# DistributedML/Biscotti

Measured on AMD Instinct MI355X. Metric: Multi-Krum GB/s (device-resident, n fp64 updates x d) + selected-set parity, higher is better.
Workload: dtype f64; 1 GPU; D_512x1M_f153; n=512, d=1048576, f=153, m=359, parallelism=1 GPU, d_local=1048576

## Files before the change

### biscotti_amd/csrc/bk_kernels.hip

```cpp
#include <hip/hip_runtime.h>
#include <stdint.h>
#include <stdlib.h>
#include <string.h>
#include <type_traits>

#include "bk_device.h"
#include "bk_internal.h"
#include "bk_synth.h"

namespace bk {

typedef float f2v __attribute__((ext_vector_type(2)));
typedef double d4v __attribute__((ext_vector_type(4)));


__device__ __forceinline__ int xcd_remap(int b, int nwg) {
    const int q = nwg >> 3, r = nwg & 7, x = b & 7;
    return (x < r ? x * (q + 1) : r * (q + 1) + (x - r) * q) + (b >> 3);
}

__device__ __forceinline__ void tri_decode(int u, int T, int &bi, int &bj) {
    int i = 0, off = 0;
    while (u >= off + (T - i)) { off += T - i; ++i; }
    bi = i;
// ... 224 lines not shown
    case 11: asm volatile("s_waitcnt vmcnt(11)" ::: "memory"); break;
    default: asm volatile("s_waitcnt vmcnt(12)" ::: "memory"); break;
    }
}

template <int N>
__device__ __forceinline__ void g3_waitc() {
    asm volatile("s_waitcnt vmcnt(%0)" ::"n"(N) : "memory");
}

__device__ __forceinline__ void g3_barrier() {
    __builtin_amdgcn_s_barrier();
    asm volatile("" ::: "memory");
    __builtin_amdgcn_sched_barrier(0);
}

__device__ __forceinline__ constexpr int dix(int i, int j) { return i * 4 - i * (i - 1) / 2 + (j - i); }

template <int KIND, typename V>
struct G3Acc;
template <typename V>
struct G3Acc<T_OFF, V> {
    V a[4][4];
};
template <typename V>
struct G3Acc<T_PAIR, V> {
    V a[10], b[10];
};
template <typename V>
struct G3Acc<T_DIAG1, V> {
    V a[10];
};

template <typename T, bool SKIP = false>
__device__ __forceinline__ void diag_mma(typename G3T<T>::acc (&acc)[10], const d2v (&a)[4]) {
    typedef typename G3T<T>::op O;
#pragma unroll
    for (int s = 0; s < 2; ++s)
#pragma unroll
        for (int i = 0; i < 4; ++i)
#pragma unroll
            for (int j = i; j < 4; ++j) {
                if (SKIP && i == 0 && j == 3) continue;
                acc[dix(i, j)] = G3T<T>::mma((O)a[i][s], (O)a[j][s], acc[dix(i, j)]);
            }
}
template <typename T>
__device__ __forceinline__ void off_mma_tail(typename G3T<T>::acc (&acc)[4][4], const d2v (&a)[4],
                                             const d2v (&b)[4]) {
    typedef typename G3T<T>::op O;
#pragma unroll
    for (int s = 0; s < 2; ++s)
#pragma unroll
        for (int i = 0; i < 4; ++i)
#pragma unroll
            for (int j = 0; j < 4; ++j) acc[i][j] = G3T<T>::mma((O)a[i][s], (O)b[j][s], acc[i][j]);
}
template <typename T, bool SKIP = false>
__device__ __forceinline__ void diag_mma_g(typename G3T<T>::acc (&acc)[10],
                                           const typename G3T<T>::gran (&a)[4]) {
#pragma unroll
    for (int s = 0; s < G3T<T>::SUB; ++s) {
        typename G3T<T>::op v[4];
#pragma unroll
        for (int i = 0; i < 4; ++i) v[i] = G3T<T>::at(a[i], s);
#pragma unroll
        for (int i = 0; i < 4; ++i)
#pragma unroll
            for (int j = i; j < 4; ++j) {
                if (SKIP && i == 0 && j == 3) continue;
                acc[dix(i, j)] = G3T<T>::mma(v[i], v[j], acc[dix(i, j)]);
            }
    }
}

template <typename T>
__device__ __forceinline__ void g3_load_rows(d2v (&a)[4], const T *__restrict__ X, int64_t ld,
                                             int n, int b, int64_t c, int64_t d, int rr) {
#pragma unroll
    for (int q = 0; q < 4; ++q) {
        const T *pr = X + (int64_t)min(b * 64 + q * 16 + rr, n - 1) * ld;
        a[q].x = c < d ? (double)pr[c] : 0.0;
        a[q].y = c + 1 < d ? (double)pr[c + 1] : 0.0;
    }
}

template <typename T = double>
__device__ __forceinline__ void store_tile(double *out, const typename G3T<T>::acc (&acc)[4][4],
                                           int rr, int g, bool wt = false) {
#pragma unroll
    for (int i = 0; i < 4; ++i)
#pragma unroll
        for (int j = 0; j < 4; ++j)
#pragma unroll
            for (int r = 0; r < 4; ++r)
                st_part(&out[(i * 16 + g3_crow<T>(g, r)) * 64 + j * 16 + rr], (double)acc[i][j][r], wt);
}

template <typename T, bool SKIP = false>
__device__ __forceinline__ void store_diag(double *out, const typename G3T<T>::acc (&acc)[10],
                                           int rr, int g, bool wt = false) {
#pragma unroll
    for (int i = 0; i < 4; ++i)
#pragma unroll
        for (int j = 0; j < 4; ++j) {
            if (SKIP && i == 0 && j == 3) continue;
#pragma unroll
            for (int r = 0; r < 4; ++r)
                st_part(&out[(i * 16 + g3_crow<T>(g, r)) * 64 + j * 16 + rr],
                        j >= i ? (double)acc[dix(i, j)][r] : 0.0, wt);
        }
}

template <typename T, int S, int XT = 0>
__device__ __forceinline__ void off_mma(typename G3T<T>::acc (&acc)[4][4],
                                        const typename G3T<T>::gran (&a)[4],
                                        const typename G3T<T>::gran (&b)[4],
                                        typename G3T<T>::acc &x) {
    typename G3T<T>::op va[4], vb[4];
#pragma unroll
    for (int i = 0; i < 4; ++i) {
        va[i] = G3T<T>::at(a[i], S);
        vb[i] = G3T<T>::at(b[i], S);
    }
#pragma unroll
    for (int i = 0; i < 4; ++i)
#pragma unroll
        for (int j = 0; j < 4; ++j)
            acc[i][j] = G3T<T>::mma(va[i], vb[j], acc[i][j]);
    if constexpr (XT == 1) x = G3T<T>::mma(va[0], va[3], x);
    if constexpr (XT == 2) x = G3T<T>::mma(vb[0], vb[3], x);
}
template <typename T, int XT = 0>
__device__ __forceinline__ void off_mma_gran(typename G3T<T>::acc (&acc)[4][4],
                                             const typename G3T<T>::gran (&a)[4],
                                             const typename G3T<T>::gran (&b)[4],
                                             typename G3T<T>::acc &x) {
    off_mma<T, 0, XT>(acc, a, b, x);
    off_mma<T, 1, XT>(acc, a, b, x);
    if constexpr (G3T<T>::SUB == 4) {
        off_mma<T, 2, XT>(acc, a, b, x);
        off_mma<T, 3, XT>(acc, a, b, x);
    }
}
#ifdef BK_K1_PROBE
#define G3_PROBE(v) const long long v = (long long)__builtin_readcyclecounter()
#else
#define G3_PROBE(v) const long long v = 0
#endif
template <typename T, int KIND, int MODE, bool STAG, int NB, int XT = 0>
__device__ __forceinline__ void g3_wave(const T *__restrict__ X, int64_t ld, int n, int nfull,
                                        int64_t d, const GroupDesc &G, const int *wd, char *lds,
                                        int wave, int lane, double *out, long long (&probe)[2],
                                        double *xout = nullptr, bool wt = false) {
    constexpr int XO = KIND == T_OFF ? XT : 0;
    constexpr bool XP = KIND == T_PAIR && XT != 0;
    typedef typename G3T<T>::gran gran;
    constexpr int EPG = 16 / (int)sizeof(T);
    constexpr int BKE = 8 * EPG;
    const int rr = lane & 15, g = lane >> 4;
    int blk[G3_MAXB];
#pragma unroll
    for (int b = 0; b < G3_MAXB; ++b) blk[b] = G.blk[b];
    const int c = NB > 0 ? NB : G.nb;
    const int sA = G.task[wave][1], sB = G.task[wave][2];
    const int kst = wd[1], kstr = wd[2], kend = wd[3];
    const int nk = kst < kend ? (kend - 1 - kst) / kstr + 1 : 0;

#ifndef BK_GLDS_E6
#define BK_GLDS_E6 2
#endif
#ifndef BK_GLDS_E4
#define BK_GLDS_E4 2
#endif
    constexpr int ESPL = G3T<T>::F32C ? 0 : NB == 6 ? BK_GLDS_E6 : NB == 4 ? BK_GLDS_E4 : 0;
    constexpr int CLO = NB + ESPL, CHI = NB - ESPL;
    constexpr int GMAX = G3_MAXB + 2;
    static_assert(CLO <= GMAX && CHI >= 0, "glds split exceeds the per-wave pointer table");
    const bool hi = wave >= 4;
    const T *gsrc[GMAX];
    int gdst[GMAX];
    {
        const int rq = lane >> 3, j = lane & 7;
#pragma unroll
        for (int m = 0; m < GMAX; ++m) {
            int i = wave + 8 * m;
            if constexpr (ESPL != 0) {
                i = hi ? 4 * CLO + (wave - 4) + 4 * m : wave + 4 * m;
                if (i >= 8 * NB) i = 0;
            }
            const int b = i >> 3, ii = i & 7;
            const int rl = ii * 8 + rq;
#ifdef BK_K1_SAMEROWS
            const int grow = min(rl, n - 1);
#else
            const int grow = min(blk[b] * 64 + rl, n - 1);
#endif
            gsrc[m] = X + (int64_t)grow * ld + EPG * (j ^ (rl & 7));
            gdst[m] = b * G3_BLK + ii * 1024;
        }
    }
    auto issue = [&](int64_t kb, int stage) {
#ifdef BK_K1_L2WINDOW
        const int64_t col = (kb % BK_K1_L2WINDOW) * BKE;
#else
        const int64_t col = kb * BKE;
#endif
        char *base = lds + stage * G3_STAGE;
#ifndef BK_K1_GLDS_LIMIT
#define BK_K1_GLDS_LIMIT G3_MAXB
#endif
        if constexpr (ESPL != 0) {
            if (hi) {
#pragma unroll
                for (int m = 0; m < CHI; ++m)
                    __builtin_amdgcn_global_load_lds((const void *)(gsrc[m] + col),
                                                     (void *)(base + gdst[m]), 16, 0, 0);
            } else {
#pragma unroll
                for (int m = 0; m < CLO; ++m)
                    __builtin_amdgcn_global_load_lds((const void *)(gsrc[m] + col),
                                                     (void *)(base + gdst[m]), 16, 0, 0);
            }
            return;
        }
#pragma unroll
        for (int m = 0; m < (NB > 0 ? NB : G3_MAXB); ++m)
            if ((NB > 0 || m < c) && m < BK_K1_GLDS_LIMIT)
                __builtin_amdgcn_global_load_lds((const void *)(gsrc[m] + col),
                                                 (void *)(base + gdst[m]), 16, 0, 0);
    };

    typedef typename G3T<T>::acc AV;
    G3Acc<KIND == T_NONE ? T_DIAG1 : KIND, AV> acc;
    if constexpr (KIND == T_OFF) {
#pragma unroll
        for (int i = 0; i < 4; ++i)
#pragma unroll
            for (int j = 0; j < 4; ++j) acc.a[i][j] = AV{0, 0, 0, 0};
    } else if constexpr (KIND == T_PAIR) {
#pragma unroll
        for (int i = 0; i < 10; ++i) acc.a[i] = acc.b[i] = AV{0, 0, 0, 0};
    } else if constexpr (KIND == T_DIAG1) {
#pragma unroll
        for (int i = 0; i < 10; ++i) acc.a[i] = AV{0, 0, 0, 0};
    }
    AV xacc = AV{0, 0, 0, 0};
    gran ha[4], hb[4];
#pragma unroll
    for (int q = 0; q < 4; ++q) ha[q] = hb[q] = gran{};

#pragma unroll
    for (int s = 0; s < G3_STAGES - 1; ++s)
        if (s < nk && MODE != 2) issue(kst + (int64_t)s * kstr, s);
    int buf = 0;
    for (int t = 0; t < nk; ++t) {
        const int ahead = min(nk - t - 1, G3_STAGES - 2);
        G3_PROBE(p0);
        if constexpr (NB > 0 && MODE != 2 && ESPL != 0) {
            if (ahead > 0) {
                if (hi)
                    g3_waitc<CHI>();
                else
                    g3_waitc<CLO>();
            } else {
                g3_waitc<0>();
            }
        } else if constexpr (NB > 0 && MODE != 2) {
            if (ahead > 0)
                g3_waitc<(NB < BK_K1_GLDS_LIMIT ? NB : BK_K1_GLDS_LIMIT)>();
            else
                g3_waitc<0>();
        } else {
            g3_wait(MODE == 2 ? 0 : ahead * c);
        }
        G3_PROBE(p1);
        g3_barrier();
        G3_PROBE(p2);
        probe[0] += p1 - p0;
        probe[1] += p2 - p1;
        const char *ls = lds + buf * G3_STAGE;
        const int nbuf = buf == 0 ? G3_STAGES - 1 : buf - 1;
        const bool more = t + G3_STAGES - 1 < nk && MODE != 2;
        const int64_t nkb = kst + (int64_t)(t + G3_STAGES - 1) * kstr;
        buf = buf == G3_STAGES - 1 ? 0 : buf + 1;
        if constexpr (MODE == 1) {
            if (more) issue(nkb, nbuf);
            continue;
        }
        if constexpr (KIND == T_OFF) {
            gran a0[4], b0[4], a1[4], b1[4];
#pragma unroll
            for (int q = 0; q < 4; ++q) a0[q] = g3_frag<T>(ls + sA * G3_BLK, q, 0, rr, g);
#pragma unroll
            for (int q = 0; q < 4; ++q) b0[q] = g3_frag<T>(ls + sB * G3_BLK, q, 0, rr, g);
            if constexpr (STAG) {
                if (t > 0) off_mma_gran<T, XO>(acc.a, ha, hb, xacc);
            }
#pragma unroll
            for (int q = 0; q < 4; ++q) a1[q] = g3_frag<T>(ls + sA * G3_BLK, q, 1, rr, g);
#pragma unroll
            for (int q = 0; q < 4; ++q) b1[q] = g3_frag<T>(ls + sB * G3_BLK, q, 1, rr, g);
            if (more) issue(nkb, nbuf);
            off_mma_gran<T, XO>(acc.a, a0, b0, xacc);
            if constexpr (STAG) {
#pragma unroll
                for (int q = 0; q < 4; ++q) {
                    ha[q] = a1[q];
                    hb[q] = b1[q];
                }
            } else {
                off_mma_gran<T, XO>(acc.a, a1, b1, xacc);
            }
        } else if constexpr (KIND == T_PAIR) {
#pragma unroll
            for (int h = 0; h < 2; ++h) {
                gran a[4], b[4];
#pragma unroll
                for (int q = 0; q < 4; ++q) a[q] = g3_frag<T>(ls + sA * G3_BLK, q, h, rr, g);
#pragma unroll
                for (int q = 0; q < 4; ++q) b[q] = g3_frag<T>(ls + sB * G3_BLK, q, h, rr, g);
                if (h == 0 && more) issue(nkb, nbuf);
                diag_mma_g<T, XP>(acc.a, a);
                diag_mma_g<T, XP>(acc.b, b);
            }
        } else if constexpr (KIND == T_DIAG1) {
#pragma unroll
            for (int h = 0; h < 2; ++h) {
                gran a[4];
#pragma unroll
                for (int q = 0; q < 4; ++q) a[q] = g3_frag<T>(ls + sA * G3_BLK, q, h, rr, g);
                if (h == 0 && more) issue(nkb, nbuf);
                diag_mma_g<T>(acc.a, a);
            }
        } else {
            if (more) issue(nkb, nbuf);
        }
    }
    if constexpr (KIND == T_OFF && STAG && MODE != 1)
        if (nk > 0) off_mma_gran<T, XO>(acc.a, ha, hb, xacc);
    if constexpr (KIND != T_NONE) {
        const int64_t c0 = (int64_t)nfull * BKE;
        if (wd[4] && c0 < d) {
#pragma unroll
            for (int h = 0; h < BKE / 8; ++h) {
                const int64_t cc = c0 + 8 * h + 2 * g;
                d2v a[4], b[4];
                g3_load_rows<T>(a, X, ld, n, blk[sA], cc, d, rr);
                g3_load_rows<T>(b, X, ld, n, blk[sB], cc, d, rr);
                if constexpr (KIND == T_OFF) {
                    typedef typename G3T<T>::op O;
                    off_mma_tail<T>(acc.a, a, b);
#pragma unroll
                    for (int s2 = 0; s2 < 2; ++s2) {
                        if constexpr (XO == 1) xacc = G3T<T>::mma((O)a[0][s2], (O)a[3][s2], xacc);
                        if constexpr (XO == 2) xacc = G3T<T>::mma((O)b[0][s2], (O)b[3][s2], xacc);
                    }
                } else if constexpr (KIND == T_PAIR) {
                    diag_mma<T, XP>(acc.a, a);
                    diag_mma<T, XP>(acc.b, b);
                } else {
                    diag_mma<T>(acc.a, a);
                }
            }
        }
        if constexpr (KIND == T_OFF) {
            store_tile<T>(out, acc.a, rr, g, wt);
            if constexpr (XO != 0) {
#pragma unroll
                for (int r = 0; r < 4; ++r)
                    st_part(&xout[g3_crow<T>(g, r) * 64 + 48 + rr], (double)xacc[r], wt);
            }
        } else if constexpr (KIND == T_PAIR) {
            store_diag<T, XP>(out, acc.a, rr, g, wt);
            store_diag<T, XP>(out + 4096, acc.b, rr, g, wt);
        } else {
            store_diag<T>(out, acc.a, rr, g, wt);
        }
    }
}

#ifndef G3_STAGGER
#define G3_STAGGER 1
#endif
template <typename T, int MODE, int NB>
__device__ __forceinline__ void g3_dispatch(const T *__restrict__ X, int64_t ld, int n,
                                            int nfull, int64_t d, const GroupDesc &G,
                                            const int *wd, char *lds, int wave, int lane,
                                            double *out, long long (&probe)[2], bool wt) {
    const int xt = (NB == 4 || NB == 0) ? G.xt[wave] : 0;
    double *xout = out - (int64_t)wave * 2 * 4096 + (int64_t)G.xslot[wave] * 4096;
    switch (G.task[wave][0]) {
    case T_OFF:
#ifndef BK_F32_STAGGER
#define BK_F32_STAGGER 0
#endif
        if (wave >= 4 && G3_STAGGER && (!G3T<T>::F32C || BK_F32_STAGGER)) {
            if (xt == 1)
                g3_wave<T, T_OFF, MODE, true, NB, (NB == 4 || NB == 0) ? 1 : 0>(X, ld, n, nfull, d, G, wd, lds, wave, lane, out, probe, xout, wt);
            else if (xt == 2)
                g3_wave<T, T_OFF, MODE, true, NB, (NB == 4 || NB == 0) ? 2 : 0>(X, ld, n, nfull, d, G, wd, lds, wave, lane, out, probe, xout, wt);
            else
                g3_wave<T, T_OFF, MODE, true, NB>(X, ld, n, nfull, d, G, wd, lds, wave, lane, out, probe, nullptr, wt);
        } else {
            if (xt == 1)
                g3_wave<T, T_OFF, MODE, false, NB, (NB == 4 || NB == 0) ? 1 : 0>(X, ld, n, nfull, d, G, wd, lds, wave, lane, out, probe, xout, wt);
            else if (xt == 2)
                g3_wave<T, T_OFF, MODE, false, NB, (NB == 4 || NB == 0) ? 2 : 0>(X, ld, n, nfull, d, G, wd, lds, wave, lane, out, probe, xout, wt);
            else
                g3_wave<T, T_OFF, MODE, false, NB>(X, ld, n, nfull, d, G, wd, lds, wave, lane, out, probe, nullptr, wt);
        }
        break;
    case T_PAIR:
        if (xt)
            g3_wave<T, T_PAIR, MODE, false, NB, (NB == 4 || NB == 0) ? 1 : 0>(X, ld, n, nfull, d, G, wd, lds, wave, lane, out, probe, nullptr, wt);
        else
            g3_wave<T, T_PAIR, MODE, false, NB>(X, ld, n, nfull, d, G, wd, lds, wave, lane, out, probe, nullptr, wt);
        break;
    case T_DIAG1:
        g3_wave<T, T_DIAG1, MODE, false, NB>(X, ld, n, nfull, d, G, wd, lds, wave, lane, out, probe, nullptr, wt);
        break;
    default:
        g3_wave<T, T_NONE, MODE, false, NB>(X, ld, n, nfull, d, G, wd, lds, wave, lane, out, probe, nullptr, wt);
        break;
    }
}
template <int MODE, typename T = double>
__global__ __launch_bounds__(512, 2) void k_gram3(const T *__restrict__ X, int64_t ld, int n,
                                                  int nfull, int64_t d,
                                                  const GroupDesc *__restrict__ groups,
                                                  const int *__restrict__ segtab,
                                                  const int *__restrict__ wgtab,
                                                  double *__restrict__ part,
                                                  long long *__restrict__ trace, PieceMarks pm) {
    extern __shared__ __attribute__((aligned(16))) char lds[];
    const int wave = __builtin_amdgcn_readfirstlane(threadIdx.x >> 6), lane = threadIdx.x & 63;
    long long t_rt0 = 0, t_mt0 = 0;
    if (trace && threadIdx.x == 0) {
        t_rt0 = (long long)__builtin_amdgcn_s_memrealtime();
        t_mt0 = (long long)__builtin_amdgcn_s_memtime();
    }
    long long probe[2] = {0, 0};
    const bool wt = piece_handed(pm) && !pm.nowt;
    const int v0 = segtab[2 * blockIdx.x], nseg = segtab[2 * blockIdx.x + 1];
    long long ideal = 0;
    for (int sg = 0; sg < nseg; ++sg) {
        const int v = v0 + sg;
        const int *wd = wgtab + 5 * v;
        const GroupDesc &G = groups[wd[0]];
        double *out = part + ((int64_t)v * 16 + wave * 2) * 4096;
        if (sg > 0) __syncthreads();
        if constexpr (MODE == 0) {
            switch (G.nb) {
            case 1: g3_dispatch<T, MODE, 1>(X, ld, n, nfull, d, G, wd, lds, wave, lane, out, probe, wt); break;
            case 2: g3_dispatch<T, MODE, 2>(X, ld, n, nfull, d, G, wd, lds, wave, lane, out, probe, wt); break;
            case 3: g3_dispatch<T, MODE, 3>(X, ld, n, nfull, d, G, wd, lds, wave, lane, out, probe, wt); break;
            case 4: g3_dispatch<T, MODE, 4>(X, ld, n, nfull, d, G, wd, lds, wave, lane, out, probe, wt); break;
            case 5: g3_dispatch<T, MODE, 5>(X, ld, n, nfull, d, G, wd, lds, wave, lane, out, probe, wt); break;
            default: g3_dispatch<T, MODE, 6>(X, ld, n, nfull, d, G, wd, lds, wave, lane, out, probe, wt); break;
            }
        } else {
            g3_dispatch<T, MODE, 0>(X, ld, n, nfull, d, G, wd, lds, wave, lane, out, probe, wt);
        }
        if (trace) ideal += (long long)(wd[1] < wd[3] ? (wd[3] - 1 - wd[1]) / wd[2] + 1 : 0) * G.cost;
    }
    piece_done(pm);
    if (trace) {
#ifdef BK_K1_PROBE
        if (lane == 0) {
            trace[24 * blockIdx.x + 8 + wave] = probe[0];
            trace[24 * blockIdx.x + 16 + wave] = probe[1];
        }
#endif
        __syncthreads();
        if (threadIdx.x == 0) {
            unsigned hw, xcc;
            asm volatile("s_getreg_b32 %0, hwreg(HW_REG_HW_ID)" : "=s"(hw));
            asm volatile("s_getreg_b32 %0, hwreg(HW_REG_XCC_ID)" : "=s"(xcc));
            long long *tr = trace + 24 * blockIdx.x;
            tr[0] = t_rt0;
            tr[1] = (long long)__builtin_amdgcn_s_memrealtime();
            tr[2] = t_mt0;
            tr[3] = (long long)__builtin_amdgcn_s_memtime();
            tr[4] = hw;
            tr[5] = xcc;
            const int g0 = nseg > 0 ? wgtab[5 * v0] : 0;
            const int c0 = groups[g0].cost > 0 ? groups[g0].cost : 1;
            tr[6] = g0 | ((long long)c0 << 32);
            tr[7] = (ideal + c0 / 2) / c0;
        }
    }
}

__global__ __launch_bounds__(256) void k_reduce3(const double *__restrict__ part,
                                                 const int *__restrict__ red,
                                                 const int *__restrict__ wglist,
                                                 double *__restrict__ U, int64_t usz,
                                                 double dcols, double dcols32, int u0, int rec) {
    if (rec && blockIdx.x == 0 && threadIdx.x == 0) {
        U[usz] = dcols;
        U[usz + 1] = dcols32;
        U[usz + 2] = 0.0;
        U[usz + 3] = 0.0;
    }
#ifndef BK_REDUCE_V1
    __shared__ d2v sub[8][32];
    const int u = u0 + (blockIdx.x >> 6), el = threadIdx.x & 31, q = threadIdx.x >> 5;
    const int e = (blockIdx.x & 63) * 64 + el * 2;
    const int off = red[3 * u], np = red[3 * u + 1], slot = red[3 * u + 2];
    const int *wl = wglist + off;
    d2v acc = {0.0, 0.0};
    int s = q;
    for (; s + 56 < np; s += 64) {
        d2v v[8];
#pragma unroll
        for (int k = 0; k < 8; ++k)
            v[k] = *reinterpret_cast<const d2v *>(part + ((int64_t)wl[s + 8 * k] * 16 + slot) * 4096 + e);
#pragma unroll
        for (int k = 0; k < 8; ++k) {
            acc.x += v[k].x;
            acc.y += v[k].y;
        }
    }
    for (; s < np; s += 8) {
        const d2v v = *reinterpret_cast<const d2v *>(part + ((int64_t)wl[s] * 16 + slot) * 4096 + e);
        acc.x += v.x;
        acc.y += v.y;
    }
    sub[q][el] = acc;
    __syncthreads();
    if (q == 0) {
        d2v t = sub[0][el];
#pragma unroll
        for (int k = 1; k < 8; ++k) {
            t.x += sub[k][el].x;
            t.y += sub[k][el].y;
        }
        *reinterpret_cast<d2v *>(U + (int64_t)u * 4096 + e) = t;
    }
#else
    __shared__ double sub[8][32];
    const int u = u0 + (blockIdx.x >> 7), el = threadIdx.x & 31, q = threadIdx.x >> 5;
    const int e = (blockIdx.x & 127) * 32 + el;
    const int off = red[3 * u], np = red[3 * u + 1], slot = red[3 * u + 2];
    const int *wl = wglist + off;
    double acc = 0.0;
    int s = q;
    for (; s + 24 < np; s += 32) {
        const double v0 = part[((int64_t)wl[s + 0] * 16 + slot) * 4096 + e];
        const double v1 = part[((int64_t)wl[s + 8] * 16 + slot) * 4096 + e];
        const double v2 = part[((int64_t)wl[s + 16] * 16 + slot) * 4096 + e];
        const double v3 = part[((int64_t)wl[s + 24] * 16 + slot) * 4096 + e];
        acc += v0;
        acc += v1;
        acc += v2;
        acc += v3;
    }
    for (; s < np; s += 8) acc += part[((int64_t)wl[s] * 16 + slot) * 4096 + e];
    sub[q][el] = acc;
    __syncthreads();
    if (q == 0) {
        double t = sub[0][el];
#pragma unroll
        for (int k = 1; k < 8; ++k) t += sub[k][el];
        U[(int64_t)u * 4096 + e] = t;
    }
#endif
}

__global__ __launch_bounds__(256) void k_reduce(const double *__restrict__ part, int ntile, int S,
                                                double *__restrict__ U, double dcols) {
    if (blockIdx.x == 0 && threadIdx.x == 0) {
        U[(int64_t)ntile * 4096] = dcols;
        U[(int64_t)ntile * 4096 + 1] = 0.0;
        U[(int64_t)ntile * 4096 + 2] = 0.0;
        U[(int64_t)ntile * 4096 + 3] = 0.0;
    }
    const int u = blockIdx.x >> 4, chunk = blockIdx.x & 15;
    const int e = chunk * 256 + threadIdx.x;
    const double *p = part + (int64_t)u * 4096 + e;
    const int64_t stride = (int64_t)ntile * 4096;
    double acc = 0.0;
    int s = 0;
    for (; s + 4 <= S; s += 4) {
        const double v0 = p[(s + 0) * stride], v1 = p[(s + 1) * stride];
        const double v2 = p[(s + 2) * stride], v3 = p[(s + 3) * stride];
        acc += v0;
        acc += v1;
        acc += v2;
        acc += v3;
    }
    for (; s < S; ++s) acc += p[s * stride];
    U[(int64_t)u * 4096 + e] = acc;
}

__global__ __launch_bounds__(256) void k_sum_ranks(const double *__restrict__ Ug, int R,
                                                   int64_t stride, double *__restrict__ U) {
    const int64_t e = (int64_t)blockIdx.x * 256 + threadIdx.x;
    if (e >= stride) return;
    double acc = 0.0;
    for (int r = 0; r < R; ++r) acc += Ug[(int64_t)r * stride + e];
    U[e] = acc;
}

template <int NT>
__global__ __launch_bounds__(NT) void k_scores(const double *__restrict__ U, int T_, int n,
                                               int npow2, int64_t k, double *__restrict__ scores,
                                               double *__restrict__ diag) {
    extern __shared__ __attribute__((aligned(16))) uint64_t keys[];
    __shared__ double red[NT / 64];
    const int i = blockIdx.x, tid = threadIdx.x;
    const double di = u_at(U, T_, i, i);
    if (tid == 0) diag[i] = di;
    for (int j = tid; j < npow2; j += NT) {
        uint64_t key = ~0ULL;
// ... 694 lines not shown
                                                      double *__restrict__ rec) {
    const int i = (int)blockIdx.x * 256 + (int)threadIdx.x;
    if (i < n) scores[i] = sg[i + i / ch];
    if (blockIdx.x != 0) return;
    __shared__ int bad;
    if (threadIdx.x == 0) bad = 0;
    __syncthreads();
    for (int p = (int)threadIdx.x; p < parts; p += 256)
        if (sg[(int64_t)p * (ch + 1) + ch] != 0.0) bad = 1;
    __syncthreads();
    if (threadIdx.x < 3) rec[threadIdx.x] = bad ? __builtin_nan("") : dcols[threadIdx.x];
}

hipError_t launch_split_unpack(const double *sg, int64_t ch, int parts, int n, const double *dcols,
                               double *scores, double *rec, hipStream_t st) {
    hipLaunchKernelGGL(k_split_unpack, dim3((unsigned)((n + 255) / 256)), dim3(256), 0, st, sg, ch,
                       parts, n, dcols, scores, rec);
    return hipGetLastError();
}

hipError_t launch_compact(const int *mask, int n, int64_t *sel, const double *diag,
                          const double *bnd, const double *dcols, int64_t k, double *margin,
                          hipStream_t st) {
    hipLaunchKernelGGL(k_compact, dim3(1), dim3(1024), 0, st, mask, n, sel, diag, bnd, dcols, k,
                       margin);
    return hipGetLastError();
}

template <bool ACCUM>
static hipError_t launch_colsum(const void *X, int dtype, int64_t ld, int64_t d, const int64_t *sel,
                                int m, double *mean, int num_cu, hipStream_t st);

template <bool SEG>
static hipError_t launch_mean_seg(const void *X, int dtype, int64_t ld, int64_t d,
                                  const int64_t *sel, int m, double *out, int num_cu, hipStream_t st);

hipError_t launch_mean(const void *X, int dtype, int64_t ld, int64_t d, const int64_t *sel, int m,
                       double *mean, int num_cu, hipStream_t st, double *seg_part) {
    const int S = mean_segments(m);
    if (S <= 1 || !seg_part) return launch_colsum<false>(X, dtype, ld, d, sel, m, mean, num_cu, st);
    hipError_t e = launch_mean_seg<true>(X, dtype, ld, d, sel, m, seg_part, num_cu, st);
    if (e != hipSuccess) return e;
    int64_t b = (d + 255) / 256;
    if (b > (int64_t)num_cu * 8) b = (int64_t)num_cu * 8;
    if (b < 1) b = 1;
    hipLaunchKernelGGL(k_mean_comb, dim3((unsigned)b), dim3(256), 0, st, seg_part, S, d, m, mean);
    return hipGetLastError();
}

template <bool SEG>
static hipError_t launch_mean_seg(const void *X, int dtype, int64_t ld, int64_t d,
                                  const int64_t *sel, int m, double *out, int num_cu, hipStream_t st) {
    const int S = mean_segments(m);
    const size_t lds = (size_t)MEAN_SEG_ROWS * sizeof(int64_t);
    const int64_t cap = ((int64_t)num_cu * 16 + S - 1) / S;
    const dim3 block(256);
    if (dtype != 0 && (ld % 4) == 0 && ((uintptr_t)X % 16) == 0) {
        int64_t b4 = ((d + 3) / 4 + 255) / 256;
        b4 = b4 > cap ? cap : b4 < 1 ? 1 : b4;
        hipLaunchKernelGGL((k_mean_f4<false, true>), dim3((unsigned)b4, (unsigned)S), block, lds, st,
                           (const float *)X, ld, d, sel, m, out);
        return hipGetLastError();
    }
    int64_t b = ((d + 1) / 2 + 255) / 256;
    b = b > cap ? cap : b < 1 ? 1 : b;
    const dim3 grid((unsigned)b, (unsigned)S);
    const bool vec = dtype == 0 ? ((ld % 2) == 0 && ((uintptr_t)X % 16) == 0)
                                : ((ld % 2) == 0 && ((uintptr_t)X % 8) == 0);
    if (dtype == 0) {
        if (vec)
            hipLaunchKernelGGL((k_mean<double, true, false, true>), grid, block, lds, st, (const double *)X,
                               ld, d, sel, m, out);
        else
            hipLaunchKernelGGL((k_mean<double, false, false, true>), grid, block, lds, st, (const double *)X,
                               ld, d, sel, m, out);
    } else {
        if (vec)
            hipLaunchKernelGGL((k_mean<float, true, false, true>), grid, block, lds, st, (const float *)X, ld,
                               d, sel, m, out);
        else
            hipLaunchKernelGGL((k_mean<float, false, false, true>), grid, block, lds, st, (const float *)X, ld,
                               d, sel, m, out);
    }
    return hipGetLastError();
}

hipError_t launch_accumulate(const void *X, int dtype, int64_t ld, int64_t d, const int64_t *idx,
                             int m, double *global, int num_cu, hipStream_t st) {
    return launch_colsum<true>(X, dtype, ld, d, idx, m, global, num_cu, st);
}

template <bool ACCUM>
static hipError_t launch_colsum(const void *X, int dtype, int64_t ld, int64_t d, const int64_t *sel,
                                int m, double *mean, int num_cu, hipStream_t st) {
    const int64_t npair = (d + 1) / 2;
    int64_t blocks = (npair + 255) / 256;
    const int64_t cap = (int64_t)num_cu * 16;
    if (blocks > cap) blocks = cap;
    if (blocks < 1) blocks = 1;
    const size_t lds = (size_t)m * sizeof(int64_t);
    const bool vec = dtype == 0 ? ((ld % 2) == 0 && ((uintptr_t)X % 16) == 0)
                                : ((ld % 2) == 0 && ((uintptr_t)X % 8) == 0);
    dim3 grid((unsigned)blocks), block(256);
    if (dtype != 0 && (ld % 4) == 0 && ((uintptr_t)X % 16) == 0) {
        int64_t b4 = ((d + 3) / 4 + 255) / 256;
        if (b4 > (int64_t)num_cu * 16) b4 = (int64_t)num_cu * 16;
        if (b4 < 1) b4 = 1;
        hipLaunchKernelGGL((k_mean_f4<ACCUM>), dim3((unsigned)b4), block, lds, st, (const float *)X, ld,
                           d, sel, m, mean);
        return hipGetLastError();
    }
    if (dtype == 0) {
        if (vec)
            hipLaunchKernelGGL((k_mean<double, true, ACCUM>), grid, block, lds, st, (const double *)X, ld, d,
                               sel, m, mean);
        else
            hipLaunchKernelGGL((k_mean<double, false, ACCUM>), grid, block, lds, st, (const double *)X, ld,
                               d, sel, m, mean);
    } else {
        if (vec)
            hipLaunchKernelGGL((k_mean<float, true, ACCUM>), grid, block, lds, st, (const float *)X, ld, d,
                               sel, m, mean);
        else
            hipLaunchKernelGGL((k_mean<float, false, ACCUM>), grid, block, lds, st, (const float *)X, ld, d,
                               sel, m, mean);
    }
    return hipGetLastError();
}

hipError_t launch_synth(void *X, int dtype, int64_t ld, int64_t n, int64_t dl, int64_t c0,
                        const int64_t *perm, const SynthParams &P, hipStream_t st) {
    int64_t bx = (dl + 255) / 256;
    if (bx > 4096) bx = 4096;
    if (bx < 1) bx = 1;
    dim3 grid((unsigned)bx, (unsigned)n), block(256);
    if (dtype == 0)
        hipLaunchKernelGGL(k_synth<double>, grid, block, 0, st, (double *)X, ld, dl, c0, perm, P);
    else
        hipLaunchKernelGGL(k_synth<float>, grid, block, 0, st, (float *)X, ld, dl, c0, perm, P);
    return hipGetLastError();
}

hipError_t launch_gram3(const void *X, int dtype, int64_t ld, int n, int64_t d, const Plan3 &pl0,
                        double *part, hipStream_t st, int mode, long long *trace, bool f32_mfma,
                        const int *seg, int nwg, const PieceMarks &pm) {
    (void)mode;
    Plan3 pl = pl0;
    if (seg) {
        pl.d_seg = const_cast<int *>(seg);
        pl.nwg = nwg;
    }
    if (pl.nwg < 1) return hipSuccess;
    const dim3 grid((unsigned)pl.nwg), block(512);
    if (dtype != 0 && f32_mfma)
        hipLaunchKernelGGL((k_gram3<0, f32m>), grid, block, G3_LDS, st, (const f32m *)X, ld, n,
                           pl.nfull, d, pl.d_groups, pl.d_seg, pl.d_wg, part, trace, pm);
    else if (dtype != 0)
        hipLaunchKernelGGL((k_gram3<0, float>), grid, block, G3_LDS, st, (const float *)X, ld, n,
                           pl.nfull, d, pl.d_groups, pl.d_seg, pl.d_wg, part, trace, pm);
#ifdef BK_PROBES
    else if (mode == 1)
        hipLaunchKernelGGL(k_gram3<1>, grid, block, G3_LDS, st, (const double *)X, ld, n, pl.nfull,
                           d, pl.d_groups, pl.d_seg, pl.d_wg, part, trace, pm);
    else if (mode == 2)
        hipLaunchKernelGGL(k_gram3<2>, grid, block, G3_LDS, st, (const double *)X, ld, n, pl.nfull,
                           d, pl.d_groups, pl.d_seg, pl.d_wg, part, trace, pm);
#endif
    else
        hipLaunchKernelGGL(k_gram3<0>, grid, block, G3_LDS, st, (const double *)X, ld, n, pl.nfull,
                           d, pl.d_groups, pl.d_seg, pl.d_wg, part, trace, pm);
    return hipGetLastError();
}

hipError_t launch_reduce3(const double *part, const Plan3 &pl, double *U, hipStream_t st,
                          bool f32_mfma, int u0, int u1, bool rec) {
    const int64_t usz = (int64_t)pl.ntile * 4096;
    const double d32 = f32_mfma ? (double)pl.d : 0.0;
    if (u1 < 0) u1 = pl.ntile;
    if (u1 <= u0) return hipSuccess;
#ifndef BK_REDUCE_V1
    hipLaunchKernelGGL(k_reduce3, dim3((unsigned)(u1 - u0) * 64), dim3(256), 0, st, part, pl.d_red,
                       pl.d_wglist, U, usz, (double)pl.d, d32, u0, rec ? 1 : 0);
#else
    hipLaunchKernelGGL(k_reduce3, dim3((unsigned)(u1 - u0) * 128), dim3(256), 0, st, part, pl.d_red,
                       pl.d_wglist, U, usz, (double)pl.d, d32, u0, rec ? 1 : 0);
#endif
    return hipGetLastError();
}

hipError_t configure_kernels() {
    for (const void *k : {(const void *)k_gram3<0>, (const void *)k_gram3<0, float>,
                          (const void *)k_gram3<0, f32m>}) {
        hipError_t e0 = hipFuncSetAttribute(k, hipFuncAttributeMaxDynamicSharedMemorySize, G3_LDS);
        if (e0 != hipSuccess) return e0;
    }
#ifdef BK_PROBES
    for (const void *k : {(const void *)k_gram3<1>, (const void *)k_gram3<2>}) {
        hipError_t e0 = hipFuncSetAttribute(k, hipFuncAttributeMaxDynamicSharedMemorySize, G3_LDS);
        if (e0 != hipSuccess) return e0;
    }
#endif
    hipError_t e = hipFuncSetAttribute((const void *)k_scores<1024>,
                                       hipFuncAttributeMaxDynamicSharedMemorySize, 131072);
    if (e != hipSuccess) return e;
    e = hipFuncSetAttribute((const void *)k_scores<256>, hipFuncAttributeMaxDynamicSharedMemorySize,
                            131072);
    if (e != hipSuccess) return e;
    for (const void *kk : {(const void *)k_scores2<256, 16, 1024, false>,
                           (const void *)k_scores2<512, 16, 1024, false>,
                           (const void *)k_scores2<1024, 16, 1024, false>,
                           (const void *)k_scores2<1024, 4, 1024, false>,
                           (const void *)k_scores2<256, 16, 1024, true>,
                           (const void *)k_scores2<512, 16, 1024, true>,
                           (const void *)k_scores2<1024, 16, 1024, true>,
                           (const void *)k_scores2<1024, 4, 1024, true>,
#ifdef BK_PROBES
                           (const void *)k_scores2<256, 16, 1024, false, 1>,
                           (const void *)k_scores2<512, 16, 1024, false, 1>,
                           (const void *)k_scores2<1024, 16, 1024, false, 1>,
                           (const void *)k_scores2<1024, 4, 1024, false, 1>,
                           (const void *)k_scores2<256, 16, 1024, false, 2>,
                           (const void *)k_scores2<512, 16, 1024, false, 2>,
                           (const void *)k_scores2<1024, 16, 1024, false, 2>,
                           (const void *)k_scores2<1024, 4, 1024, false, 2>,
                           (const void *)k_scores2<256, 16, 1024, true, 1>,
                           (const void *)k_scores2<512, 16, 1024, true, 1>,
                           (const void *)k_scores2<1024, 16, 1024, true, 1>,
                           (const void *)k_scores2<1024, 4, 1024, true, 1>,
                           (const void *)k_scores2<256, 16, 1024, true, 2>,
                           (const void *)k_scores2<512, 16, 1024, true, 2>,
                           (const void *)k_scores2<1024, 16, 1024, true, 2>,
                           (const void *)k_scores2<1024, 4, 1024, true, 2>,
#endif
                       }) {
        e = hipFuncSetAttribute(kk, hipFuncAttributeMaxDynamicSharedMemorySize, 144 * 1024);
        if (e != hipSuccess) return e;
    }
    for (const void *k : {(const void *)k_mean<double, true, false>,
                          (const void *)k_mean<double, false, false>,
                          (const void *)k_mean<float, true, false>,
                          (const void *)k_mean<float, false, false>,
                          (const void *)k_mean<double, true, true>,
                          (const void *)k_mean<double, false, true>,
                          (const void *)k_mean<float, true, true>,
                          (const void *)k_mean<float, false, true>,
                          (const void *)k_mean_f4<false>, (const void *)k_mean_f4<true>}) {
        e = hipFuncSetAttribute(k, hipFuncAttributeMaxDynamicSharedMemorySize, 131072);
        if (e != hipSuccess) return e;
    }
    return hipSuccess;
}

}
```

Measured before the change: 935.4 GB/s.

## Use scalar row bases with a shared 32-bit lane offset for global-to-LDS loads

Replaces the per-lane 64-bit source pointer table (one per load slot) with per-slot scalar row bases plus a single 32-bit per-lane voffset, which cuts VGPR use and address arithmetic in the load-issue loop. A slow path that clamps rows per lane is kept for ragged edge blocks, for strides too large for a 32-bit offset, or when an env var forces it. The split of global_load_lds work between low and high waves for NB=4/6 also changes from 2 to 3. This adds runtime branching and relies on the 32-bit offset assumption holding.

```diff
diff --git a/biscotti_amd/csrc/bk_kernels.hip b/biscotti_amd/csrc/bk_kernels.hip
--- a/biscotti_amd/csrc/bk_kernels.hip
+++ b/biscotti_amd/csrc/bk_kernels.hip
@@ -400,7 +400,7 @@
 __device__ __forceinline__ void g3_wave(const T *__restrict__ X, int64_t ld, int n, int nfull,
                                         int64_t d, const GroupDesc &G, const int *wd, char *lds,
                                         int wave, int lane, double *out, long long (&probe)[2],
-                                        double *xout = nullptr, bool wt = false) {
+                                        double *xout, bool wt, bool perlane) {
     constexpr int XO = KIND == T_OFF ? XT : 0;
     constexpr bool XP = KIND == T_PAIR && XT != 0;
     typedef typename G3T<T>::gran gran;
@@ -416,67 +416,82 @@
     const int nk = kst < kend ? (kend - 1 - kst) / kstr + 1 : 0;
 
 #ifndef BK_GLDS_E6
-#define BK_GLDS_E6 2
+#define BK_GLDS_E6 3
 #endif
 #ifndef BK_GLDS_E4
-#define BK_GLDS_E4 2
+#define BK_GLDS_E4 3
 #endif
     constexpr int ESPL = G3T<T>::F32C ? 0 : NB == 6 ? BK_GLDS_E6 : NB == 4 ? BK_GLDS_E4 : 0;
     constexpr int CLO = NB + ESPL, CHI = NB - ESPL;
-    constexpr int GMAX = G3_MAXB + 2;
-    static_assert(CLO <= GMAX && CHI >= 0, "glds split exceeds the per-wave pointer table");
+    static_assert(ESPL >= 0 && CHI >= 0, "glds split moves more loads than waves 4-7 have");
+    static_assert(G3_BLK == 8 * 1024, "LDS byte of instruction i is 1024 i");
+    constexpr int SLOTS = ESPL != 0 ? CLO : NB > 0 ? NB : G3_MAXB;
+    constexpr int ISTEP = ESPL != 0 ? 4 : 8;
     const bool hi = wave >= 4;
-    const T *gsrc[GMAX];
-    int gdst[GMAX];
-    {
-        const int rq = lane >> 3, j = lane & 7;
-#pragma unroll
-        for (int m = 0; m < GMAX; ++m) {
-            int i = wave + 8 * m;
-            if constexpr (ESPL != 0) {
-                i = hi ? 4 * CLO + (wave - 4) + 4 * m : wave + 4 * m;
-                if (i >= 8 * NB) i = 0;
-            }
-            const int b = i >> 3, ii = i & 7;
-            const int rl = ii * 8 + rq;
+    const int i0 = (ESPL != 0 && hi) ? 4 * CLO + (wave - 4) : wave;
+    const int rq = lane >> 3, j = lane & 7;
+    const uint32_t voff = (uint32_t)rq * (uint32_t)(ld * (int64_t)sizeof(T)) + 16u * (uint32_t)(j ^ rq);
+    int srow[SLOTS];
+    const char *sbase[SLOTS];
+#pragma unroll
+    for (int m = 0; m < SLOTS; ++m) {
+        int i = i0 + ISTEP * m;
+        if (ESPL != 0 && i >= 8 * NB) i = 0;
+        const int b = i >> 3, ii = i & 7;
 #ifdef BK_K1_SAMEROWS
-            const int grow = min(rl, n - 1);
+        srow[m] = ii * 8;
 #else
-            const int grow = min(blk[b] * 64 + rl, n - 1);
+        srow[m] = G.blk[b] * 64 + ii * 8;
 #endif
-            gsrc[m] = X + (int64_t)grow * ld + EPG * (j ^ (rl & 7));
-            gdst[m] = b * G3_BLK + ii * 1024;
-        }
-    }
+        sbase[m] = (const char *)X + (int64_t)srow[m] * ld * (int64_t)sizeof(T);
+    }
+    bool slow = perlane;
+#ifndef BK_K1_SAMEROWS
+#pragma unroll
+    for (int b = 0; b < (NB > 0 ? NB : G3_MAXB); ++b)
+        if ((NB > 0 || b < c) && blk[b] * 64 + 64 > n) slow = true;
+#endif
+#ifndef BK_K1_GLDS_LIMIT
+#define BK_K1_GLDS_LIMIT G3_MAXB
+#endif
+    auto each_slot = [&](auto &&f) {
+        if constexpr (ESPL != 0) {
+            if (hi) {
+#pragma unroll
+                for (int m = 0; m < CHI; ++m) f(m);
+            } else {
+#pragma unroll
+                for (int m = 0; m < CLO; ++m) f(m);
+            }
+        } else {
+#pragma unroll
+            for (int m = 0; m < SLOTS; ++m)
+                if ((NB > 0 || m < c) && m < BK_K1_GLDS_LIMIT) f(m);
+        }
+    };
     auto issue = [&](int64_t kb, int stage) {
 #ifdef BK_K1_L2WINDOW
         const int64_t col = (kb % BK_K1_L2WINDOW) * BKE;
 #else
         const int64_t col = kb * BKE;
 #endif
-        char *base = lds + stage * G3_STAGE;
-#ifndef BK_K1_GLDS_LIMIT
-#define BK_K1_GLDS_LIMIT G3_MAXB
-#endif
-        if constexpr (ESPL != 0) {
-            if (hi) {
-#pragma unroll
-                for (int m = 0; m < CHI; ++m)
-                    __builtin_amdgcn_global_load_lds((const void *)(gsrc[m] + col),
-                                                     (void *)(base + gdst[m]), 16, 0, 0);
-            } else {
-#pragma unroll
-                for (int m = 0; m < CLO; ++m)
-                    __builtin_amdgcn_global_load_lds((const void *)(gsrc[m] + col),
-                                                     (void *)(base + gdst[m]), 16, 0, 0);
-            }
-            return;
-        }
-#pragma unroll
-        for (int m = 0; m < (NB > 0 ? NB : G3_MAXB); ++m)
-            if ((NB > 0 || m < c) && m < BK_K1_GLDS_LIMIT)
-                __builtin_amdgcn_global_load_lds((const void *)(gsrc[m] + col),
-                                                 (void *)(base + gdst[m]), 16, 0, 0);
+        char *base = lds + stage * G3_STAGE + i0 * 1024;
+        if (slow) {
+            int rqs = rq;
+            asm volatile("" : "+v"(rqs));
+            each_slot([&](int m) {
+                const int grow = min(srow[m] + rqs, n - 1);
+                const T *src = X + (int64_t)grow * ld + EPG * (j ^ rq) + col;
+                __builtin_amdgcn_global_load_lds((const void *)src,
+                                                 (void *)(base + m * ISTEP * 1024), 16, 0, 0);
+            });
+        } else {
+            const uint32_t vo = voff + (uint32_t)(col * (int64_t)sizeof(T));
+            each_slot([&](int m) {
+                __builtin_amdgcn_global_load_lds((const void *)(sbase[m] + (uint64_t)vo),
+                                                 (void *)(base + m * ISTEP * 1024), 16, 0, 0);
+            });
+        }
     };
 
     typedef typename G3T<T>::acc AV;
@@ -635,7 +650,8 @@
 __device__ __forceinline__ void g3_dispatch(const T *__restrict__ X, int64_t ld, int n,
                                             int nfull, int64_t d, const GroupDesc &G,
                                             const int *wd, char *lds, int wave, int lane,
-                                            double *out, long long (&probe)[2], bool wt) {
+                                            double *out, long long (&probe)[2], bool wt,
+                                            bool perlane) {
     const int xt = (NB == 4 || NB == 0) ? G.xt[wave] : 0;
     double *xout = out - (int64_t)wave * 2 * 4096 + (int64_t)G.xslot[wave] * 4096;
     switch (G.task[wave][0]) {
@@ -645,31 +661,31 @@
 #endif
         if (wave >= 4 && G3_STAGGER && (!G3T<T>::F32C || BK_F32_STAGGER)) {
             if (xt == 1)
-                g3_wave<T, T_OFF, MODE, true, NB, (NB == 4 || NB == 0) ? 1 : 0>(X, ld, n, nfull, d, G, wd, lds, wave, lane, out, probe, xout, wt);
+                g3_wave<T, T_OFF, MODE, true, NB, (NB == 4 || NB == 0) ? 1 : 0>(X, ld, n, nfull, d, G, wd, lds, wave, lane, out, probe, xout, wt, perlane);
             else if (xt == 2)
-                g3_wave<T, T_OFF, MODE, true, NB, (NB == 4 || NB == 0) ? 2 : 0>(X, ld, n, nfull, d, G, wd, lds, wave, lane, out, probe, xout, wt);
+                g3_wave<T, T_OFF, MODE, true, NB, (NB == 4 || NB == 0) ? 2 : 0>(X, ld, n, nfull, d, G, wd, lds, wave, lane, out, probe, xout, wt, perlane);
             else
-                g3_wave<T, T_OFF, MODE, true, NB>(X, ld, n, nfull, d, G, wd, lds, wave, lane, out, probe, nullptr, wt);
+                g3_wave<T, T_OFF, MODE, true, NB>(X, ld, n, nfull, d, G, wd, lds, wave, lane, out, probe, nullptr, wt, perlane);
         } else {
             if (xt == 1)
-                g3_wave<T, T_OFF, MODE, false, NB, (NB == 4 || NB == 0) ? 1 : 0>(X, ld, n, nfull, d, G, wd, lds, wave, lane, out, probe, xout, wt);
+                g3_wave<T, T_OFF, MODE, false, NB, (NB == 4 || NB == 0) ? 1 : 0>(X, ld, n, nfull, d, G, wd, lds, wave, lane, out, probe, xout, wt, perlane);
             else if (xt == 2)
-                g3_wave<T, T_OFF, MODE, false, NB, (NB == 4 || NB == 0) ? 2 : 0>(X, ld, n, nfull, d, G, wd, lds, wave, lane, out, probe, xout, wt);
+                g3_wave<T, T_OFF, MODE, false, NB, (NB == 4 || NB == 0) ? 2 : 0>(X, ld, n, nfull, d, G, wd, lds, wave, lane, out, probe, xout, wt, perlane);
             else
-                g3_wave<T, T_OFF, MODE, false, NB>(X, ld, n, nfull, d, G, wd, lds, wave, lane, out, probe, nullptr, wt);
+                g3_wave<T, T_OFF, MODE, false, NB>(X, ld, n, nfull, d, G, wd, lds, wave, lane, out, probe, nullptr, wt, perlane);
         }
         break;
     case T_PAIR:
         if (xt)
-            g3_wave<T, T_PAIR, MODE, false, NB, (NB == 4 || NB == 0) ? 1 : 0>(X, ld, n, nfull, d, G, wd, lds, wave, lane, out, probe, nullptr, wt);
+            g3_wave<T, T_PAIR, MODE, false, NB, (NB == 4 || NB == 0) ? 1 : 0>(X, ld, n, nfull, d, G, wd, lds, wave, lane, out, probe, nullptr, wt, perlane);
         else
-            g3_wave<T, T_PAIR, MODE, false, NB>(X, ld, n, nfull, d, G, wd, lds, wave, lane, out, probe, nullptr, wt);
+            g3_wave<T, T_PAIR, MODE, false, NB>(X, ld, n, nfull, d, G, wd, lds, wave, lane, out, probe, nullptr, wt, perlane);
         break;
     case T_DIAG1:
-        g3_wave<T, T_DIAG1, MODE, false, NB>(X, ld, n, nfull, d, G, wd, lds, wave, lane, out, probe, nullptr, wt);
+        g3_wave<T, T_DIAG1, MODE, false, NB>(X, ld, n, nfull, d, G, wd, lds, wave, lane, out, probe, nullptr, wt, perlane);
         break;
     default:
-        g3_wave<T, T_NONE, MODE, false, NB>(X, ld, n, nfull, d, G, wd, lds, wave, lane, out, probe, nullptr, wt);
+        g3_wave<T, T_NONE, MODE, false, NB>(X, ld, n, nfull, d, G, wd, lds, wave, lane, out, probe, nullptr, wt, perlane);
         break;
     }
 }
@@ -680,7 +696,8 @@
                                                   const int *__restrict__ segtab,
                                                   const int *__restrict__ wgtab,
                                                   double *__restrict__ part,
-                                                  long long *__restrict__ trace, PieceMarks pm) {
+                                                  long long *__restrict__ trace, PieceMarks pm,
+                                                  int perlane) {
     extern __shared__ __attribute__((aligned(16))) char lds[];
     const int wave = __builtin_amdgcn_readfirstlane(threadIdx.x >> 6), lane = threadIdx.x & 63;
     long long t_rt0 = 0, t_mt0 = 0;
@@ -700,15 +717,15 @@
         if (sg > 0) __syncthreads();
         if constexpr (MODE == 0) {
             switch (G.nb) {
-            case 1: g3_dispatch<T, MODE, 1>(X, ld, n, nfull, d, G, wd, lds, wave, lane, out, probe, wt); break;
-            case 2: g3_dispatch<T, MODE, 2>(X, ld, n, nfull, d, G, wd, lds, wave, lane, out, probe, wt); break;
-            case 3: g3_dispatch<T, MODE, 3>(X, ld, n, nfull, d, G, wd, lds, wave, lane, out, probe, wt); break;
-            case 4: g3_dispatch<T, MODE, 4>(X, ld, n, nfull, d, G, wd, lds, wave, lane, out, probe, wt); break;
-            case 5: g3_dispatch<T, MODE, 5>(X, ld, n, nfull, d, G, wd, lds, wave, lane, out, probe, wt); break;
-            default: g3_dispatch<T, MODE, 6>(X, ld, n, nfull, d, G, wd, lds, wave, lane, out, probe, wt); break;
+            case 1: g3_dispatch<T, MODE, 1>(X, ld, n, nfull, d, G, wd, lds, wave, lane, out, probe, wt, perlane != 0); break;
+            case 2: g3_dispatch<T, MODE, 2>(X, ld, n, nfull, d, G, wd, lds, wave, lane, out, probe, wt, perlane != 0); break;
+            case 3: g3_dispatch<T, MODE, 3>(X, ld, n, nfull, d, G, wd, lds, wave, lane, out, probe, wt, perlane != 0); break;
+            case 4: g3_dispatch<T, MODE, 4>(X, ld, n, nfull, d, G, wd, lds, wave, lane, out, probe, wt, perlane != 0); break;
+            case 5: g3_dispatch<T, MODE, 5>(X, ld, n, nfull, d, G, wd, lds, wave, lane, out, probe, wt, perlane != 0); break;
+            default: g3_dispatch<T, MODE, 6>(X, ld, n, nfull, d, G, wd, lds, wave, lane, out, probe, wt, perlane != 0); break;
             }
         } else {
-            g3_dispatch<T, MODE, 0>(X, ld, n, nfull, d, G, wd, lds, wave, lane, out, probe, wt);
+            g3_dispatch<T, MODE, 0>(X, ld, n, nfull, d, G, wd, lds, wave, lane, out, probe, wt, perlane != 0);
         }
         if (trace) ideal += (long long)(wd[1] < wd[3] ? (wd[3] - 1 - wd[1]) / wd[2] + 1 : 0) * G.cost;
     }
@@ -1709,23 +1726,26 @@
     }
     if (pl.nwg < 1) return hipSuccess;
     const dim3 grid((unsigned)pl.nwg), block(512);
+    const int64_t rowb = ld * (dtype != 0 ? 4 : 8);
+    const char *pe = getenv("BK_TEST_GLDS_PERLANE");
+    const int perlane = (8 * rowb + 128 > (int64_t)UINT32_MAX || (pe && atoi(pe) != 0)) ? 1 : 0;
     if (dtype != 0 && f32_mfma)
         hipLaunchKernelGGL((k_gram3<0, f32m>), grid, block, G3_LDS, st, (const f32m *)X, ld, n,
-                           pl.nfull, d, pl.d_groups, pl.d_seg, pl.d_wg, part, trace, pm);
+                           pl.nfull, d, pl.d_groups, pl.d_seg, pl.d_wg, part, trace, pm, perlane);
     else if (dtype != 0)
         hipLaunchKernelGGL((k_gram3<0, float>), grid, block, G3_LDS, st, (const float *)X, ld, n,
-                           pl.nfull, d, pl.d_groups, pl.d_seg, pl.d_wg, part, trace, pm);
+                           pl.nfull, d, pl.d_groups, pl.d_seg, pl.d_wg, part, trace, pm, perlane);
 #ifdef BK_PROBES
     else if (mode == 1)
         hipLaunchKernelGGL(k_gram3<1>, grid, block, G3_LDS, st, (const double *)X, ld, n, pl.nfull,
-                           d, pl.d_groups, pl.d_seg, pl.d_wg, part, trace, pm);
+                           d, pl.d_groups, pl.d_seg, pl.d_wg, part, trace, pm, perlane);
     else if (mode == 2)
         hipLaunchKernelGGL(k_gram3<2>, grid, block, G3_LDS, st, (const double *)X, ld, n, pl.nfull,
-                           d, pl.d_groups, pl.d_seg, pl.d_wg, part, trace, pm);
+                           d, pl.d_groups, pl.d_seg, pl.d_wg, part, trace, pm, perlane);
 #endif
     else
         hipLaunchKernelGGL(k_gram3<0>, grid, block, G3_LDS, st, (const double *)X, ld, n, pl.nfull,
-                           d, pl.d_groups, pl.d_seg, pl.d_wg, part, trace, pm);
+                           d, pl.d_groups, pl.d_seg, pl.d_wg, part, trace, pm, perlane);
     return hipGetLastError();
 }
 
```

After: 936.7 GB/s, median of 5. About the same (+0.1%).
